# vllm-project/production-stack

Hardware: AMD Instinct MI355X
Metric: output_tokens_per_sec (higher is better)
Workload: dtype bfloat16; 1 GPU; multi-round-qa; model=llama-3-8b, users_per_gpu=320, rounds_per_conversation=10, max_model_len=8192, parallelism=dp1, prefix_caching=True, kv_cache_dtype=auto, quantization=none

## Files before the change

### csrc/bindings.cpp

```cpp
#include <hip/hip_runtime.h>
#include <torch/extension.h>

#include <c10/hip/HIPStream.h>

#include <algorithm>

extern "C" {
int ps_rms_norm(void* out, const void* x, const void* w, float eps, long T,
                int D, hipStream_t stream);
int ps_fused_add_rms_norm(void* x, void* residual, const void* w, float eps,
                          long T, int D, hipStream_t stream);
int ps_rms_norm_fp8(void* out_q, void* out_scale, void* x, void* residual,
                    const void* w, float eps, long T, int D, int fused,
                    hipStream_t stream);
int ps_silu_and_mul_fp8(void* out_q, void* out_scale, const void* x, long T,
                        int D, hipStream_t stream);
void ps_silu_and_mul(void* out, const void* x, long T, int D,
                     hipStream_t stream);
void ps_rope(const void* positions, void* q, void* k, const void* cos_sin,
             long T, int QH, int KH, int HD, int ROT, hipStream_t stream);
void ps_fused_rope_cache(void* qkv, const void* positions, const void* cos_sin,
                         const void* slot_mapping, void* k_cache,
                         void* v_cache, long T, int QH, int KH, int HD,
                         int ROT, long qkv_stride, int BS, int kv_fp8,
                         hipStream_t stream);
int ps_paged_attn_decode(void* out, void* ws_acc, void* ws_ml, const void* q,
                         const void* k_cache, const void* v_cache,
                         const void* block_tables, const void* seq_lens,
                         int num_seqs, int max_blocks, float scale, int KH,
                         int GQ, int head_dim, int block_size, int num_splits,
                         long q_stride, int variant, int kv_fp8, int window,
                         const void* order, hipStream_t stream);
int ps_decode_order(void* order, const void* seq_lens, int S,
                    hipStream_t stream);
int ps_prefill_mfma32_splits(int num_tiles, int KH, int GQ);
int ps_paged_attn_prefill_mfma32(void* out, void* ws_o, void* ws_ml,
                                 long q_tokens, const void* q,
                                 const void* k_cache, const void* v_cache,
                                 const void* block_tables,
                                 const void* tile_info, int num_tiles,
                                 int num_q_heads, int max_blocks,
                                 float scale, int KH, int GQ, int head_dim,
                                 long q_stride, int kv_fp8, int window,
                                 hipStream_t stream);
int ps_paged_attn_prefill_mfma(void* out, const void* q, const void* k_cache,
                               const void* v_cache, const void* block_tables,
                               const void* tile_info, int num_tiles,
                               int num_q_heads, int max_blocks, float scale,
                               int KH, int GQ, int head_dim, long q_stride,
                               int variant, int kv_fp8, int window, hipStream_t stream);
int ps_paged_attn_prefill(void* out, const void* q, const void* k_cache,
                          const void* v_cache, const void* block_tables,
                          const void* token_seq, const void* token_pos,
                          int num_tokens, int num_q_heads, int max_blocks,
                          float scale, int KH, int GQ, int head_dim,
                          int block_size, long q_stride, int window,
                          hipStream_t stream);
void ps_reshape_and_cache(const void* k, const void* v, void* k_cache,
                          void* v_cache, const void* slot_mapping, long T,
                          int KH, int HD, int BS, int kv_fp8,
                          hipStream_t stream);
void ps_greedy_sample(void* out, const void* logits, long R, int V,
                      hipStream_t stream);
void ps_kv_quant(void* out, void* scales, const void* in, long rows, int hd,
                 hipStream_t stream);
void ps_kv_dequant(void* out, const void* in, const void* scales, long rows,
                   int hd, hipStream_t stream);
int ps_skinny_gemm_splits(int M, int N, int K);
int ps_skinny_gemm(void* out_bf16, void* ws, const void* x, const void* w,
                   int M, int N, int K, long x_stride, hipStream_t stream);
int ps_skinny_gemm_fp8_splits(int M, int N, int K);
int ps_skinny_gemm_fp8(void* out_bf16, void* ws, const void* xq,
                       const void* sx, const void* wq, const void* sw, int M,
                       int N, int K, hipStream_t stream);
int ps_quant_fp8_rows(void* out_q, void* out_scale, const void* x, long T,
                      int D, long x_stride, hipStream_t stream);
int ps_gemm8p_splits(int M, int N, int K);
int ps_gemm8p(void* out_bf16, void* ws, const void* x, const void* w, int M,
              int N, int K, long x_stride, hipStream_t stream);
int ps_lora_bgmv(void* out, const void* x, const void* A, const void* B,
                 const void* scale, const void* idx, int T, int IN, int W,
                 int R, long out_stride, long x_stride, int col_off,
                 hipStream_t stream);
int ps_fused_moe_supported(int T, int top_k, int E, int H, int I);
int ps_fused_moe(void* out, void* offsets, void* sorted_pairs, void* act,
                 void* y, const void* x, const void* w_gate_up,
                 const void* w_down, const void* topk_ids, int ids_i64,
                 const void* topk_w, int T, int top_k, int E, int H, int I,
                 hipStream_t stream);
}

at::Tensor cachegen_encode(at::Tensor q);
at::Tensor cachegen_decode(at::Tensor blob, int64_t hd);

namespace {

hipStream_t current_stream() {
  return c10::hip::getCurrentHIPStream().stream();
}

#define CHECK_GPU_BF16(t)                                             \
  TORCH_CHECK((t).is_cuda(), #t " must be on the GPU");               \
  TORCH_CHECK((t).scalar_type() == at::kBFloat16, #t " must be bf16"); \
  TORCH_CHECK((t).is_contiguous(), #t " must be contiguous")

#define CHECK_GPU_DTYPE(t, ty)                                  \
  TORCH_CHECK((t).is_cuda(), #t " must be on the GPU");         \
  TORCH_CHECK((t).scalar_type() == (ty), #t " dtype mismatch"); \
  TORCH_CHECK((t).is_contiguous(), #t " must be contiguous")

void check_fp8_outputs(const at::Tensor& out_q, const at::Tensor& scales,
                       long T, long D) {
  TORCH_CHECK(out_q.is_cuda() && out_q.is_contiguous(),
              "out_q must be GPU-contiguous");
  TORCH_CHECK(out_q.scalar_type() == at::kFloat8_e4m3fn ||
                  out_q.scalar_type() == at::kByte,
              "out_q must be fp8/byte");
  TORCH_CHECK(out_q.dim() == 2 && out_q.size(0) == T && out_q.size(1) == D,
              "out_q must be [", T, ", ", D, "]");
  CHECK_GPU_DTYPE(scales, at::kFloat);
  TORCH_CHECK(scales.numel() == T, "scales must hold one value per row");
}

int rotary_dim(const at::Tensor& cos_sin, int HD) {
  TORCH_CHECK(cos_sin.dim() == 2, "cos_sin must be [max_pos, rot_dim]");
  const long ROT = cos_sin.size(1);
  TORCH_CHECK(ROT >= 0 && ROT % 2 == 0, "rot_dim must be even, got ", ROT);
// ... 101 lines not shown
  const int QH = (int)q.size(1);
  const int HD = (int)q.size(2);
  const int KH = (int)k_cache.size(1);
  const int BS = (int)k_cache.size(2);
  TORCH_CHECK(QH % KH == 0, "GQA group mismatch");
  const int GQ = QH / KH;
  const int max_blocks = (int)block_tables.size(1);
  if (num_splits <= 0) {
    const int target = 2048;
    num_splits = std::min<int64_t>(
        32, std::max<int64_t>(1, target / std::max(1, S * KH)));
  }
  at::Tensor ws_acc, ws_ml;
  void *acc_p = nullptr, *ml_p = nullptr;
  if (num_splits > 1) {
    auto opts = q.options().dtype(at::kFloat);
    ws_acc = at::empty({(long)S * QH * num_splits * HD}, opts);
    ws_ml = at::empty({(long)S * QH * num_splits * 2}, opts);
    acc_p = ws_acc.data_ptr();
    ml_p = ws_ml.data_ptr();
  }
  int rc = ps_paged_attn_decode(
      out.data_ptr(), acc_p, ml_p, q.data_ptr(), k_cache.data_ptr(),
      v_cache.data_ptr(), block_tables.data_ptr(), seq_lens.data_ptr(), S,
      max_blocks, (float)scale, KH, GQ, HD, BS, (int)num_splits,
      q_row_stride(q, HD), (int)variant, kv_fp8, (int)window, order_p,
      current_stream());
  TORCH_CHECK(rc == 0, "unsupported decode config: head_dim=", HD,
              " block_size=", BS, " gqa=", GQ, " variant=", variant);
}

bool decode_order(at::Tensor order, at::Tensor seq_lens) {
  CHECK_GPU_DTYPE(order, at::kInt);
  CHECK_GPU_DTYPE(seq_lens, at::kInt);
  TORCH_CHECK(order.numel() == seq_lens.numel(), "order/seq_lens size");
  return ps_decode_order(order.data_ptr(), seq_lens.data_ptr(),
                         (int)seq_lens.numel(), current_stream()) == 0;
}

void paged_attn_prefill(at::Tensor out, at::Tensor q, at::Tensor k_cache,
                        at::Tensor v_cache, at::Tensor block_tables,
                        at::Tensor token_seq, at::Tensor token_pos,
                        double scale, int64_t window) {
  CHECK_GPU_BF16(out);
  CHECK_GPU_BF16(k_cache);
  CHECK_GPU_BF16(v_cache);
  CHECK_GPU_DTYPE(block_tables, at::kInt);
  CHECK_GPU_DTYPE(token_seq, at::kInt);
  CHECK_GPU_DTYPE(token_pos, at::kInt);
  const int T = (int)q.size(0);
  const int QH = (int)q.size(1);
  const int HD = (int)q.size(2);
  const int KH = (int)k_cache.size(1);
  const int BS = (int)k_cache.size(2);
  TORCH_CHECK(QH % KH == 0, "GQA group mismatch");
  const int GQ = QH / KH;
  const int max_blocks = (int)block_tables.size(1);
  int rc = ps_paged_attn_prefill(
      out.data_ptr(), q.data_ptr(), k_cache.data_ptr(), v_cache.data_ptr(),
      block_tables.data_ptr(), token_seq.data_ptr(), token_pos.data_ptr(), T,
      QH, max_blocks, (float)scale, KH, GQ, HD, BS, q_row_stride(q, HD),
      (int)window, current_stream());
  TORCH_CHECK(rc == 0, "unsupported prefill config: head_dim=", HD,
              " block_size=", BS);
}

void paged_attn_prefill_mfma(at::Tensor out, at::Tensor q,
                             at::Tensor k_cache, at::Tensor v_cache,
                             at::Tensor block_tables, at::Tensor tile_info,
                             double scale, int64_t variant, int64_t window) {
  CHECK_GPU_BF16(out);
  const int kv_fp8 = cache_fp8(k_cache);
  cache_fp8(v_cache);
  CHECK_GPU_DTYPE(block_tables, at::kInt);
  CHECK_GPU_DTYPE(tile_info, at::kInt);
  const int QH = (int)q.size(1);
  const int HD = (int)q.size(2);
  const int KH = (int)k_cache.size(1);
  TORCH_CHECK(QH % KH == 0, "GQA group mismatch");
  TORCH_CHECK(k_cache.size(2) == 16, "mfma prefill needs block_size 16");
  const int GQ = QH / KH;
  const int NT = (int)tile_info.size(0);
  int rc;
  if (variant == 5) {
    const int splits = ps_prefill_mfma32_splits(NT, KH, QH / KH);
    const long T = q.size(0);
    void *ws_o_p = nullptr, *ws_ml_p = nullptr;
    at::Tensor ws_o, ws_ml;
    if (splits > 1) {
      ws_o = at::empty({(long)splits * T * QH * HD},
                       q.options().dtype(at::kFloat));
      ws_ml = at::empty({2L * splits * T * QH},
                        q.options().dtype(at::kFloat));
      ws_o_p = ws_o.data_ptr();
      ws_ml_p = ws_ml.data_ptr();
    }
    rc = ps_paged_attn_prefill_mfma32(
        out.data_ptr(), ws_o_p, ws_ml_p, T, q.data_ptr(),
        k_cache.data_ptr(), v_cache.data_ptr(), block_tables.data_ptr(),
        tile_info.data_ptr(), NT, QH, (int)block_tables.size(1),
        (float)scale, KH, QH / KH, HD, q_row_stride(q, HD), kv_fp8,
        (int)window, current_stream());
  } else {
    rc = ps_paged_attn_prefill_mfma(
        out.data_ptr(), q.data_ptr(), k_cache.data_ptr(),
        v_cache.data_ptr(), block_tables.data_ptr(), tile_info.data_ptr(),
        NT, QH, (int)block_tables.size(1), (float)scale, KH, GQ, HD,
        q_row_stride(q, HD), (int)variant, kv_fp8, (int)window,
        current_stream());
  }
  TORCH_CHECK(rc == 0, "unsupported mfma prefill config: head_dim=", HD);
}

void fused_rope_cache(at::Tensor qkv, at::Tensor positions,
                      at::Tensor cos_sin, at::Tensor slot_mapping,
                      at::Tensor k_cache, at::Tensor v_cache,
                      int64_t q_heads, int64_t head_dim) {
  CHECK_GPU_BF16(qkv);
  CHECK_GPU_DTYPE(positions, at::kInt);
  CHECK_GPU_DTYPE(cos_sin, at::kFloat);
  CHECK_GPU_DTYPE(slot_mapping, at::kLong);
  const int kv_fp8 = cache_fp8(k_cache);
  cache_fp8(v_cache);
  const long T = positions.numel();
  TORCH_CHECK(k_cache.dim() == 4 && v_cache.sizes() == k_cache.sizes() &&
                  v_cache.scalar_type() == k_cache.scalar_type(),
              "k/v cache must both be [NB, KH, BS, HD] of one dtype");
  const int KH = (int)k_cache.size(1);
  const int BS = (int)k_cache.size(2);
  TORCH_CHECK(head_dim > 0 && head_dim % 8 == 0,
              "head_dim must be a positive multiple of 8");
  const int HD = (int)head_dim;
  TORCH_CHECK(k_cache.size(3) == HD, "cache head_dim mismatch");
  const int ROT = rotary_dim(cos_sin, HD);
  TORCH_CHECK(qkv.dim() == 2 && qkv.size(0) == T &&
                  qkv.size(1) == (q_heads + 2 * KH) * HD,
              "qkv must be [T, (q_heads + 2*KH) * head_dim]");
  TORCH_CHECK(slot_mapping.numel() == T, "one slot per token");
  if (T == 0) return;
  ps_fused_rope_cache(qkv.data_ptr(), positions.data_ptr(),
                      cos_sin.data_ptr(), slot_mapping.data_ptr(),
                      k_cache.data_ptr(), v_cache.data_ptr(), T,
                      (int)q_heads, KH, HD, ROT, qkv.stride(0), BS, kv_fp8,
                      current_stream());
}

void reshape_and_cache(at::Tensor k, at::Tensor v, at::Tensor k_cache,
                       at::Tensor v_cache, at::Tensor slot_mapping) {
  CHECK_GPU_BF16(k);
  CHECK_GPU_BF16(v);
  const int kv_fp8 = cache_fp8(k_cache);
  cache_fp8(v_cache);
  CHECK_GPU_DTYPE(slot_mapping, at::kLong);
  const long T = slot_mapping.numel();
  TORCH_CHECK(k_cache.dim() == 4 && v_cache.sizes() == k_cache.sizes() &&
                  v_cache.scalar_type() == k_cache.scalar_type(),
              "k/v cache must both be [NB, KH, BS, HD] of one dtype");
  const int KH = (int)k_cache.size(1);
  const int BS = (int)k_cache.size(2);
  const int HD = (int)k_cache.size(3);
  TORCH_CHECK(HD % 8 == 0, "head_dim must be a multiple of 8");
  TORCH_CHECK(k.numel() == T * KH * HD, "k shape mismatch");
  TORCH_CHECK(v.numel() == T * KH * HD, "v shape mismatch");
  if (T == 0) return;
  ps_reshape_and_cache(k.data_ptr(), v.data_ptr(), k_cache.data_ptr(),
                       v_cache.data_ptr(), slot_mapping.data_ptr(), T, KH, HD,
                       BS, kv_fp8, current_stream());
}

void skinny_gemm(at::Tensor out, at::Tensor x, at::Tensor w) {
  CHECK_GPU_BF16(out);
  TORCH_CHECK(x.is_cuda() && x.scalar_type() == at::kBFloat16,
              "x must be bf16");
  TORCH_CHECK(x.dim() == 2 && x.stride(1) == 1, "x must be 2D row-major");
  CHECK_GPU_BF16(w);
  const int M = (int)x.size(0);
  const int K = (int)x.size(1);
  const int N = (int)w.size(0);
  TORCH_CHECK(w.size(1) == K, "K mismatch");
  const int splits = ps_skinny_gemm_splits(M, N, K);
  TORCH_CHECK(splits > 0, "unsupported skinny gemm shape M=", M, " N=", N,
              " K=", K);
  void* ws_p = nullptr;
  at::Tensor ws;
  if (splits > 1) {
// ... 324 lines not shown
```

### csrc/prefill_mfma.hip

```cpp
#include "ps_common.h"

typedef __attribute__((ext_vector_type(8))) __bf16 ps_mbf16x8;
typedef __attribute__((ext_vector_type(4))) float ps_mf32x4;

PS_DEV ps_mbf16x8 ps_as_mbf16(ps_bf16x8 u) {
  union {
    ps_bf16x8 u16;
    ps_mbf16x8 bf;
  } v;
  v.u16 = u;
  return v.bf;
}

#define PS_CHUNK 64
#define PS_PL_STRIDE 72

template <int HEAD_DIM, int WPS, typename KVT>
__global__ __launch_bounds__(256, WPS) void paged_attn_prefill_mfma_kernel(
    unsigned short* __restrict__ out,
    const unsigned short* __restrict__ q,
    const KVT* __restrict__ k_cache,
    const KVT* __restrict__ v_cache,
    const int* __restrict__ block_tables,
    const int* __restrict__ tile_info,
// ... 175 lines not shown
      for (int r = 0; r < 4; r++) m_new[r] = ps_group_max<16>(m_new[r]);
      constexpr float PS_RESCALE_THR = 11.54f;
      bool grew = false;
#pragma unroll
      for (int r = 0; r < 4; r++)
        grew |= (m_new[r] > m_run[r] + PS_RESCALE_THR) ||
                (m_run[r] == PS_NEG_INF && m_new[r] > PS_NEG_INF);
      if (__any(grew)) {
#pragma unroll
        for (int r = 0; r < 4; r++) {
          const float corr = exp2f(m_run[r] - m_new[r]);
          l_run[r] *= corr;
#pragma unroll
          for (int s = 0; s < 8; s++) o_acc[s][r] *= corr;
          m_run[r] = m_new[r];
        }
      }
      float psum[4] = {0.f, 0.f, 0.f, 0.f};
#pragma unroll
      for (int ct = 0; ct < NCT; ct++) {
#pragma unroll
        for (int r = 0; r < 4; r++) {
          const float p = s_frag[ct][r] > PS_NEG_INF
                              ? exp2f(s_frag[ct][r] - m_run[r])
                              : 0.f;
          s_frag[ct][r] = p;
          psum[r] += p;
        }
      }
#pragma unroll
      for (int r = 0; r < 4; r++) {
        float rs = ps_group_sum<16>(psum[r]);
        l_run[r] += rs;
      }
#pragma unroll
      for (int ct = 0; ct < NCT; ct++)
#pragma unroll
        for (int r = 0; r < 4; r++)
          p_lds[wave][g * 4 + r][ct * 16 + rc] =
              ps_f32_to_bf16(s_frag[ct][r]);
#pragma unroll
      for (int kc = 0; kc < NKC; kc++) {
        ps_mbf16x8 p_frag = ps_as_mbf16(
            *(const ps_bf16x8*)(&p_lds[wave][rc][kc * 32 + g * 8]));
        __builtin_amdgcn_s_setprio(1);
#pragma unroll
        for (int s = 0; s < 8; s++) {
          const int d = s * 16 + rc;
          const int pg2 = (kc * 4 + g) ^ (d & 7);
          ps_mbf16x8 v_frag =
              ps_as_mbf16(*(const ps_bf16x8*)(&v_t[d][pg2 << 3]));
          o_acc[s] = __builtin_amdgcn_mfma_f32_16x16x32_bf16(
              p_frag, v_frag, o_acc[s], 0, 0, 0);
        }
        __builtin_amdgcn_s_setprio(0);
      }
    }
    __syncthreads();
  }

#pragma unroll
  for (int r = 0; r < 4; r++) {
    const int lrow = wave * 16 + g * 4 + r;
    if (lrow >= n_rows) continue;
    const float inv = l_run[r] > 0.f ? 1.f / l_run[r] : 0.f;
    unsigned short* orow = out + ((long)(q_tok0 + lrow) * QH + qh) * D;
#pragma unroll
    for (int s = 0; s < 8; s++)
      orow[s * 16 + rc] = ps_f32_to_bf16(o_acc[s][r] * inv);
  }
}

extern "C" {

int ps_prefill_mfma32_splits(int num_tiles, int KH, int GQ);
int ps_paged_attn_prefill_mfma32(void* out, void* ws_o, void* ws_ml,
                                 long q_tokens, const void* q,
                                 const void* k_cache, const void* v_cache,
                                 const void* block_tables,
                                 const void* tile_info, int num_tiles,
                                 int num_q_heads, int max_blocks,
                                 float scale, int KH, int GQ, int head_dim,
                                 long q_stride, int kv_fp8, int window,
                                 hipStream_t stream);

int ps_paged_attn_prefill_mfma(void* out, const void* q, const void* k_cache,
                               const void* v_cache, const void* block_tables,
                               const void* tile_info, int num_tiles,
                               int num_q_heads, int max_blocks, float scale,
                               int KH, int GQ, int head_dim, long q_stride,
                               int variant, int kv_fp8, int window,
                               hipStream_t stream) {
  if (head_dim != 128) return -1;
  if (variant == 5) {
    return ps_paged_attn_prefill_mfma32(
        out, nullptr, nullptr, 0, q, k_cache, v_cache,
        block_tables, tile_info, num_tiles,
        num_q_heads, max_blocks, scale, KH, GQ, head_dim, q_stride,
        kv_fp8, window, stream);
  }
  const int n_work = num_tiles * num_q_heads;
  dim3 grid(((n_work + 7) / 8) * 8);
#define PS_PREFILL_T(WPS, KVT)                                              \
  paged_attn_prefill_mfma_kernel<128, WPS, KVT><<<grid, 256, 0, stream>>>(  \
      (unsigned short*)out, (const unsigned short*)q,                       \
      (const KVT*)k_cache, (const KVT*)v_cache, (const int*)block_tables,   \
      (const int*)tile_info, max_blocks, scale, KH, GQ, q_stride,           \
      num_q_heads, n_work, window)
  if (kv_fp8) {
    if (variant == 3) PS_PREFILL_T(3, unsigned char);
    else PS_PREFILL_T(4, unsigned char);
  } else {
    if (variant == 3) PS_PREFILL_T(3, unsigned short);
    else PS_PREFILL_T(4, unsigned short);
  }
#undef PS_PREFILL_T
  return 0;
}

}
```

### csrc/prefill_mfma32.hip

```cpp
#include "ps_common.h"

typedef __attribute__((ext_vector_type(8))) __bf16 ps_mbf16x8;
typedef __attribute__((ext_vector_type(16))) float ps_mf32x16;

PS_DEV ps_mbf16x8 ps_as_mbf16_32(ps_bf16x8 u) {
  union {
    ps_bf16x8 u16;
    ps_mbf16x8 bf;
  } v;
  v.u16 = u;
  return v.bf;
}

#define PS_CHUNK32 64
#define PS_TILE32 256

template <int HEAD_DIM, int GQW, typename KVT>
__global__ __launch_bounds__(512, 2) void paged_attn_prefill_mfma32_kernel(
    unsigned short* __restrict__ out,
    float* __restrict__ ws_o,
    float* __restrict__ ws_ml,
    long q_tokens,
    const unsigned short* __restrict__ q,
    const KVT* __restrict__ k_cache,
    const KVT* __restrict__ v_cache,
    const int* __restrict__ block_tables,
    const int* __restrict__ tile_info,
    int max_blocks, float scale, int KH, int GQ, long q_stride,
    int QH, int n_work, int window) {
  const int split = blockIdx.y;
  const int n_splits = gridDim.y;
  using KVTr = ps_kv_traits<KVT>;
  using kvec8 = typename KVTr::vec8;
  using kvec4 = typename KVTr::vec4;
  constexpr int D = HEAD_DIM;
  constexpr int BS = 16;
  constexpr int NKS = D / 16;
  constexpr int ROWH = 8 / GQW;

  const int W = n_work;
  const int cpx = (W + 7) >> 3;
  const int w = (blockIdx.x & 7) * cpx + (blockIdx.x >> 3);
  if (w >= W) return;
  const int n_grp = GQ / GQW;
  const int n_tiles = W / (n_grp * KH);
  const int tile = w % n_tiles;
  const int g_grp = (w / n_tiles) % n_grp;
  const int kvh = w / (n_tiles * n_grp);
  const int seq_row = tile_info[tile * 4 + 0];
  const int q_tok0 = tile_info[tile * 4 + 1];
  const int q_pos0 = tile_info[tile * 4 + 2];
  const int n_rows = tile_info[tile * 4 + 3];

  const int tid = threadIdx.x;
  const int wave = tid >> 6;
  const int lane = tid & 63;
  const int hi = lane >> 5;
  const int rc = lane & 31;
  const int qh = kvh * GQ + g_grp * GQW + (wave / ROWH);
  const int wq0 = (wave % ROWH) * 32;

  const int* bt = block_tables + (long)seq_row * max_blocks;
  const int ctx_limit = q_pos0 + n_rows;
  const int n_pages = (ctx_limit + BS - 1) / BS;
  const int n_chunks = (ctx_limit + PS_CHUNK32 - 1) / PS_CHUNK32;

  __shared__ __align__(16) unsigned short k_lds[PS_CHUNK32][D];
  __shared__ __align__(16) unsigned short v_t[D][PS_CHUNK32];
  __shared__ __align__(16) unsigned short p_lds[8][32][64];

  const int q_row_clamped = min(wq0 + rc, n_rows - 1);
  const unsigned short* qrow =
      q + (long)(q_tok0 + q_row_clamped) * q_stride + (long)qh * D;
  const float qmul = scale * 1.44269504f;
  ps_mbf16x8 q_frag[NKS];
#pragma unroll
  for (int ks = 0; ks < NKS; ks++) {
    ps_bf16x8 qv = *(const ps_bf16x8*)(qrow + ks * 16 + hi * 8);
    ps_bf16x8 qs;
#pragma unroll
    for (int j = 0; j < 8; j++)
      qs[j] = ps_f32_to_bf16(ps_bf16_to_f32(qv[j]) * qmul);
    q_frag[ks] = ps_as_mbf16_32(qs);
  }

  float m_run = PS_NEG_INF, l_run = 0.f;
  ps_mf32x16 o_acc[4];
#pragma unroll
  for (int dt = 0; dt < 4; dt++)
#pragma unroll
    for (int r = 16; r-- > 0;) o_acc[dt][r] = 0.f;

  const int q_pos = q_pos0 + wq0 + rc;
  const int wave_pos_max = q_pos0 + min(wq0 + 31, n_rows - 1);
  const int wave_win_lo =
      window > 0 ? max(0, (q_pos0 + wq0) - window + 1) : 0;

  const int ktok = tid >> 3, kslot = tid & 7;
  const int vtq = tid & 15, vds = tid >> 4;
  auto k_seg_ptr = [&](int chunk) {
    const int tok = chunk * PS_CHUNK32 + ktok;
    const long pg = bt[min(tok / BS, n_pages - 1)];
    return k_cache + ((pg * KH + kvh) * BS + (tok & (BS - 1))) * D +
           kslot * 8;
  };
  auto v_quad_ptr = [&](int chunk) {
    const int tok = chunk * PS_CHUNK32 + vtq * 4;
    const long pg = bt[min(tok / BS, n_pages - 1)];
    return v_cache + ((pg * KH + kvh) * BS + (tok & (BS - 1))) * D + vds * 4;
  };
  kvec8 kstage[2];
  kvec4 vstage[4];
  {
    const KVT* ks = k_seg_ptr(split);
    const KVT* vq = v_quad_ptr(split);
    kstage[0] = *(const kvec8*)ks;
    kstage[1] = *(const kvec8*)(ks + 64);
#pragma unroll
    for (int i = 0; i < 4; i++) vstage[i] = *(const kvec4*)(vq + i * D);
  }

  for (int chunk = split; chunk < n_chunks; chunk += n_splits) {
    const int tok0 = chunk * PS_CHUNK32;
    *(ps_bf16x8*)(&k_lds[ktok][(kslot ^ (ktok & 7)) * 8]) =
        KVTr::to_bf16x8(kstage[0]);
    *(ps_bf16x8*)(&k_lds[ktok][((kslot ^ (ktok & 7)) + 8) * 8]) =
        KVTr::to_bf16x8(kstage[1]);
    {
      const int vo = vtq >> 1;
      const int off = (vtq & 1) * 4;
#pragma unroll
      for (int dd = 0; dd < 4; dd++) {
        const int d = vds * 4 + dd;
        unsigned short r4[4];
#pragma unroll
        for (int i = 0; i < 4; i++) r4[i] = KVTr::to_bf16(vstage[i][dd]);
        *(ps_bf16x4*)(&v_t[d][(vo ^ (d & 7)) * 8 + off]) =
            *(const ps_bf16x4*)r4;
      }
    }
    __syncthreads();
    if (chunk + n_splits < n_chunks) {
      const KVT* ks = k_seg_ptr(chunk + n_splits);
      const KVT* vq = v_quad_ptr(chunk + n_splits);
      kstage[0] = *(const kvec8*)ks;
      kstage[1] = *(const kvec8*)(ks + 64);
#pragma unroll
      for (int i = 0; i < 4; i++) vstage[i] = *(const kvec4*)(vq + i * D);
    }

    const bool wave_active = (wq0 < n_rows) && (tok0 <= wave_pos_max) &&
                             (tok0 + PS_CHUNK32 > wave_win_lo);
    if (wave_active) {
      ps_mf32x16 s_frag[2];
#pragma unroll
      for (int kt = 0; kt < 2; kt++) {
#pragma unroll
        for (int r = 16; r-- > 0;) s_frag[kt][r] = 0.f;
        const int ktok_row = kt * 32 + rc;
        __builtin_amdgcn_s_setprio(1);
#pragma unroll
        for (int ks = 0; ks < NKS; ks++) {
          const int slot = ((ks * 2 + hi) ^ (ktok_row & 7));
          ps_mbf16x8 k_frag = ps_as_mbf16_32(
              *(const ps_bf16x8*)(&k_lds[ktok_row][slot * 8]));
          s_frag[kt] = __builtin_amdgcn_mfma_f32_32x32x16_bf16(
              k_frag, q_frag[ks], s_frag[kt], 0, 0, 0);
        }
        __builtin_amdgcn_s_setprio(0);
      }
      bool full_chunk = (tok0 + PS_CHUNK32 - 1 <= q_pos0 + wq0) &&
                        (wq0 + 31 < n_rows);
      if (window > 0)
        full_chunk = full_chunk && (tok0 >= wave_pos_max - window + 1);
      float m_new = m_run;
      if (full_chunk) {
#pragma unroll
        for (int kt = 0; kt < 2; kt++)
#pragma unroll
          for (int r = 0; r < 16; r++)
            m_new = fmaxf(m_new, s_frag[kt][r]);
      } else {
        const bool row_real = (wq0 + rc) < n_rows;
#pragma unroll
        for (int kt = 0; kt < 2; kt++) {
#pragma unroll
          for (int r = 0; r < 16; r++) {
            const int kv_pos =
                tok0 + kt * 32 + (r & 3) + 8 * (r >> 2) + 4 * hi;
            bool valid = row_real && (kv_pos <= q_pos);
            if (window > 0) valid = valid && (kv_pos > q_pos - window);
            const float sv = valid ? s_frag[kt][r] : PS_NEG_INF;
            s_frag[kt][r] = sv;
            m_new = fmaxf(m_new, sv);
          }
        }
      }
      m_new = fmaxf(m_new, __shfl_xor(m_new, 32));
      constexpr float PS_RESCALE_THR32 = 11.54f;
      const bool grew = (m_new > m_run + PS_RESCALE_THR32) ||
                        (m_run == PS_NEG_INF && m_new > PS_NEG_INF);
      if (__any(grew)) {
        const float corr = exp2f(m_run - m_new);
        l_run *= corr;
        m_run = m_new;
#pragma unroll
        for (int r = 0; r < 16; r++) {
          const int row = (r & 3) + 8 * (r >> 2) + 4 * hi;
          const float c = __shfl(corr, row);
#pragma unroll
          for (int dt = 0; dt < 4; dt++) o_acc[dt][r] *= c;
        }
      }
      float psum = 0.f;
#pragma unroll
      for (int kt = 0; kt < 2; kt++) {
#pragma unroll
        for (int r = 0; r < 16; r++) {
          const float p = s_frag[kt][r] > PS_NEG_INF
                              ? exp2f(s_frag[kt][r] - m_run)
                              : 0.f;
          s_frag[kt][r] = p;
          psum += p;
        }
      }
      l_run += psum + __shfl_xor(psum, 32);
#pragma unroll
      for (int kt = 0; kt < 2; kt++)
#pragma unroll
        for (int qd = 0; qd < 4; qd++) {
          unsigned short p4[4];
#pragma unroll
          for (int j = 0; j < 4; j++)
            p4[j] = ps_f32_to_bf16(s_frag[kt][qd * 4 + j]);
          const int slot = (kt * 4 + qd) ^ (rc & 7);
          *(ps_bf16x4*)(&p_lds[wave][rc][slot * 8 + 4 * hi]) =
              *(const ps_bf16x4*)p4;
        }
#pragma unroll
      for (int kc = 0; kc < 4; kc++) {
        const int pslot = ((kc * 2 + hi) ^ (rc & 7));
        ps_mbf16x8 p_frag = ps_as_mbf16_32(
            *(const ps_bf16x8*)(&p_lds[wave][rc][pslot * 8]));
        __builtin_amdgcn_s_setprio(1);
#pragma unroll
        for (int dt = 0; dt < 4; dt++) {
          const int d = dt * 32 + rc;
          const int vo = (kc * 2 + hi) ^ (d & 7);
          ps_mbf16x8 v_frag =
              ps_as_mbf16_32(*(const ps_bf16x8*)(&v_t[d][vo * 8]));
          o_acc[dt] = __builtin_amdgcn_mfma_f32_32x32x16_bf16(
              p_frag, v_frag, o_acc[dt], 0, 0, 0);
        }
        __builtin_amdgcn_s_setprio(0);
      }
    }
    __syncthreads();
  }

  if (n_splits > 1) {
    if (hi == 0 && wq0 + rc < n_rows) {
      const long t = q_tok0 + wq0 + rc;
      ws_ml[((long)split * q_tokens + t) * QH + qh] = m_run;
      ws_ml[((long)(n_splits + split) * q_tokens + t) * QH + qh] = l_run;
    }
#pragma unroll
    for (int r = 0; r < 16; r++) {
      const int row = (r & 3) + 8 * (r >> 2) + 4 * hi;
      const int lrow = wq0 + row;
      if (lrow >= n_rows) continue;
      float* orow = ws_o +
          (((long)split * q_tokens + q_tok0 + lrow) * QH + qh) * D;
#pragma unroll
      for (int dt = 0; dt < 4; dt++)
        orow[dt * 32 + rc] = o_acc[dt][r];
    }
    return;
  }

  const float inv_own = l_run > 0.f ? 1.f / l_run : 0.f;
#pragma unroll
  for (int r = 0; r < 16; r++) {
    const int row = (r & 3) + 8 * (r >> 2) + 4 * hi;
    const int lrow = wq0 + row;
    const float inv = __shfl(inv_own, row);
    if (lrow >= n_rows) continue;
    unsigned short* orow = out + ((long)(q_tok0 + lrow) * QH + qh) * D;
#pragma unroll
    for (int dt = 0; dt < 4; dt++)
      orow[dt * 32 + rc] = ps_f32_to_bf16(o_acc[dt][r] * inv);
  }
}

__global__ void prefill_split_combine_kernel(
    unsigned short* __restrict__ out,
    const float* __restrict__ ws_o,
    const float* __restrict__ ws_ml,
    long q_tokens, int QH, int n_splits) {
  const long th = blockIdx.x;
  if (th >= q_tokens * QH) return;
  const int d = threadIdx.x;
  float M = PS_NEG_INF;
  for (int s = 0; s < n_splits; s++)
    M = fmaxf(M, ws_ml[(long)s * q_tokens * QH + th]);
  float denom = 0.f, acc = 0.f;
  for (int s = 0; s < n_splits; s++) {
    const float m = ws_ml[(long)s * q_tokens * QH + th];
    const float l = ws_ml[((long)(n_splits + s) * q_tokens) * QH + th];
    const float w = (m > PS_NEG_INF && l > 0.f) ? exp2f(m - M) : 0.f;
    denom += w * l;
    acc += w * ws_o[((long)s * q_tokens * QH + th) * 128 + d];
  }
  out[th * 128 + d] =
      ps_f32_to_bf16(denom > 0.f ? acc / denom : 0.f);
}

extern "C" {

int ps_prefill_mfma32_splits(int num_tiles, int KH, int GQ) {
  int gqw = 1;
  while (gqw < 4 && GQ % (gqw * 2) == 0) gqw *= 2;
  const int n_work = num_tiles * KH * (GQ / gqw);
  if (n_work >= 500) return 1;
  int s = (500 + n_work - 1) / n_work;
  return s > 8 ? 8 : s;
}

int ps_paged_attn_prefill_mfma32(void* out, void* ws_o, void* ws_ml,
                                 long q_tokens, const void* q,
                                 const void* k_cache, const void* v_cache,
                                 const void* block_tables,
                                 const void* tile_info, int num_tiles,
                                 int num_q_heads, int max_blocks,
                                 float scale, int KH, int GQ, int head_dim,
                                 long q_stride, int kv_fp8, int window,
                                 hipStream_t stream) {
  if (head_dim != 128) return -1;
  int gqw = 1;
  while (gqw < 4 && GQ % (gqw * 2) == 0) gqw *= 2;
  const int n_work = num_tiles * KH * (GQ / gqw);
  int splits = ps_prefill_mfma32_splits(num_tiles, KH, GQ);
  if (ws_o == nullptr) splits = 1;
  dim3 grid(((n_work + 7) / 8) * 8, splits);
#define PS_PF32_LAUNCH(GQW, KVT)                                          \
  paged_attn_prefill_mfma32_kernel<128, GQW, KVT>                         \
      <<<grid, 512, 0, stream>>>(                                         \
          (unsigned short*)out, (float*)ws_o, (float*)ws_ml, q_tokens,    \
          (const unsigned short*)q,                                       \
          (const KVT*)k_cache, (const KVT*)v_cache,                       \
          (const int*)block_tables, (const int*)tile_info, max_blocks,    \
          scale, KH, GQ, q_stride, num_q_heads, n_work, window)
  if (kv_fp8) {
    if (gqw == 4) PS_PF32_LAUNCH(4, unsigned char);
    else if (gqw == 2) PS_PF32_LAUNCH(2, unsigned char);
    else PS_PF32_LAUNCH(1, unsigned char);
  } else {
    if (gqw == 4) PS_PF32_LAUNCH(4, unsigned short);
    else if (gqw == 2) PS_PF32_LAUNCH(2, unsigned short);
    else PS_PF32_LAUNCH(1, unsigned short);
  }
#undef PS_PF32_LAUNCH
  if (splits > 1) {
    prefill_split_combine_kernel<<<
        dim3((unsigned)(q_tokens * num_q_heads)), 128, 0, stream>>>(
        (unsigned short*)out, (const float*)ws_o, (const float*)ws_ml,
        q_tokens, num_q_heads, splits);
  }
  return 0;
}

}
```

### production_stack_amd/ops/__init__.py

```python

from __future__ import annotations

import os
from typing import Optional

import torch

from production_stack_amd.ops import reference

try:
    from production_stack_amd import _C
except ImportError:
    _C = None

HAVE_EXT = _C is not None


def _require_ext() -> None:
    if _C is None:
        raise RuntimeError(
            "production_stack_amd._C HIP extension is not built; run "
            "`PYTORCH_ROCM_ARCH=gfx950 python setup.py build_ext --inplace`. "
            "Refusing to fall back to eager PyTorch on GPU."
        )
# ... 79 lines not shown

DECODE_VARIANT = int(os.environ.get("PS_DECODE_VARIANT", "3"))
DECODE_ORDER = os.environ.get("PS_DECODE_ORDER", "1") != "0"


def _check_out(out: torch.Tensor, q: torch.Tensor) -> None:
    if (
        out.shape != q.shape
        or out.dtype != q.dtype
        or out.device != q.device
        or not out.is_contiguous()
    ):
        raise ValueError(
            "out must be contiguous with q's shape, dtype and device"
        )


def paged_attn_decode(
    q: torch.Tensor,
    k_cache: torch.Tensor,
    v_cache: torch.Tensor,
    block_tables: torch.Tensor,
    seq_lens: torch.Tensor,
    scale: float,
    window: int = 0,
    order: Optional[torch.Tensor] = None,
    out: Optional[torch.Tensor] = None,
    variant: Optional[int] = None,
) -> torch.Tensor:
    if out is not None:
        _check_out(out, q)
    if q.is_cuda:
        _require_ext()
        if out is None:
            out = torch.empty(q.shape, dtype=q.dtype, device=q.device)
        _C.paged_attn_decode(
            out, q, k_cache, v_cache, block_tables, seq_lens, scale, 0,
            DECODE_VARIANT if variant is None else variant, window, order
        )
        return out
    res = reference.paged_attn_decode(
        q, k_cache, v_cache, block_tables, seq_lens, scale, window
    )
    if out is None:
        return res
    out.copy_(res)
    return out


def decode_order(seq_lens: torch.Tensor) -> Optional[torch.Tensor]:
    if seq_lens.is_cuda:
        _require_ext()
        order = torch.empty_like(seq_lens)
        if not _C.decode_order(order, seq_lens):
            return None
        return order
    return torch.argsort(-seq_lens, stable=True).int()


def paged_attn_prefill(
    q: torch.Tensor,
    k_cache: torch.Tensor,
    v_cache: torch.Tensor,
    block_tables: torch.Tensor,
    token_seq: torch.Tensor,
    token_pos: torch.Tensor,
    scale: float,
    window: int = 0,
) -> torch.Tensor:
    if q.is_cuda:
        _require_ext()
        out = torch.empty(q.shape, dtype=q.dtype, device=q.device)
        _C.paged_attn_prefill(
            out, q, k_cache, v_cache, block_tables, token_seq, token_pos,
            scale, window
        )
        return out
    return reference.paged_attn_prefill(
        q, k_cache, v_cache, block_tables, token_seq, token_pos, scale,
        window
    )


PREFILL_VARIANT = int(os.environ.get("PS_PREFILL_VARIANT", "5"))


def prefill_tile_rows(num_q_heads: int, num_kv_heads: int) -> int:
    if PREFILL_VARIANT != 5:
        return 64
    gq = max(1, num_q_heads // max(1, num_kv_heads))
    gqw = 1
    while gqw < 4 and gq % (gqw * 2) == 0:
        gqw *= 2
    return 32 * (8 // gqw)


def paged_attn_prefill_mfma(
    q: torch.Tensor,
    k_cache: torch.Tensor,
    v_cache: torch.Tensor,
    block_tables: torch.Tensor,
    tile_info: torch.Tensor,
    scale: float,
    window: int = 0,
    variant: int = None,
    out: Optional[torch.Tensor] = None,
) -> torch.Tensor:
    _require_ext()
    if out is None:
        out = torch.empty(q.shape, dtype=q.dtype, device=q.device)
    else:
        _check_out(out, q)
    v = PREFILL_VARIANT if variant is None else variant
    _C.paged_attn_prefill_mfma(
        out, q, k_cache, v_cache, block_tables, tile_info, scale, v, window
    )
    return out


def greedy_sample(logits: torch.Tensor) -> torch.Tensor:
    if logits.is_cuda:
        _require_ext()
        if logits.dtype != torch.bfloat16:
            return logits.float().argmax(dim=-1)
        out = torch.empty(
            logits.shape[0], dtype=torch.long, device=logits.device
        )
        _C.greedy_sample(out, logits)
        return out
    return reference.greedy_sample(logits)


def kv_quant(x: torch.Tensor) -> tuple:
    if x.is_cuda:
        _require_ext()
        hd = x.shape[-1]
        out = torch.empty(x.shape, dtype=torch.int8, device=x.device)
        scales = torch.empty(
            x.numel() // hd, dtype=torch.float32, device=x.device
        )
        _C.kv_quant(out, scales, x)
        return out, scales
    return reference.kv_quant(x)


def kv_dequant(
    q: torch.Tensor, scales: torch.Tensor, dtype=torch.bfloat16
) -> torch.Tensor:
    if q.is_cuda:
        _require_ext()
        out = torch.empty(q.shape, dtype=dtype, device=q.device)
        _C.kv_dequant(out, q, scales)
        return out
    return reference.kv_dequant(q, scales, dtype)


def skinny_gemm(x: torch.Tensor, w: torch.Tensor) -> torch.Tensor:
    _require_ext()
    out = torch.empty(
        (x.shape[0], w.shape[0]), dtype=torch.bfloat16, device=x.device
    )
    _C.skinny_gemm(out, x, w)
    return out


def cachegen_encode(q: torch.Tensor) -> torch.Tensor:
    if _C is not None and hasattr(_C, "cachegen_encode"):
        return _C.cachegen_encode(q.contiguous().cpu())
    return reference.cachegen_encode(q)


# ... 200 lines not shown
```

Baseline: 5948 tokens/s.

## Add double-buffered prefill attention variant with register-resident P and make it default

Adds variant 6 of the 32x32 MFMA prefill attention kernel. It double-buffers the K/V shared-memory tiles so that one barrier per chunk replaces two, and overlaps staging of the next chunk with compute. It also keeps the softmax probabilities in registers by swapping the MFMA operand order, which removes the P round-trip through LDS and the per-row corr shuffles, and it uses the raw exp2 builtin. The cost is more LDS for the K/V buffers (offset by dropping p_lds), a transposed output layout, and some risk in the edge handling of -inf rows.

```diff
diff --git a/csrc/bindings.cpp b/csrc/bindings.cpp
--- a/csrc/bindings.cpp
+++ b/csrc/bindings.cpp
@@ -42,7 +42,7 @@
                                  int num_q_heads, int max_blocks,
                                  float scale, int KH, int GQ, int head_dim,
                                  long q_stride, int kv_fp8, int window,
-                                 hipStream_t stream);
+                                 int variant, hipStream_t stream);
 int ps_paged_attn_prefill_mfma(void* out, const void* q, const void* k_cache,
                                const void* v_cache, const void* block_tables,
                                const void* tile_info, int num_tiles,
@@ -310,7 +310,7 @@
   const int GQ = QH / KH;
   const int NT = (int)tile_info.size(0);
   int rc;
-  if (variant == 5) {
+  if (variant == 5 || variant == 6) {
     const int splits = ps_prefill_mfma32_splits(NT, KH, QH / KH);
     const long T = q.size(0);
     void *ws_o_p = nullptr, *ws_ml_p = nullptr;
@@ -328,7 +328,7 @@
         k_cache.data_ptr(), v_cache.data_ptr(), block_tables.data_ptr(),
         tile_info.data_ptr(), NT, QH, (int)block_tables.size(1),
         (float)scale, KH, QH / KH, HD, q_row_stride(q, HD), kv_fp8,
-        (int)window, current_stream());
+        (int)window, (int)variant, current_stream());
   } else {
     rc = ps_paged_attn_prefill_mfma(
         out.data_ptr(), q.data_ptr(), k_cache.data_ptr(),
diff --git a/csrc/prefill_mfma.hip b/csrc/prefill_mfma.hip
--- a/csrc/prefill_mfma.hip
+++ b/csrc/prefill_mfma.hip
@@ -281,7 +281,7 @@
                                  int num_q_heads, int max_blocks,
                                  float scale, int KH, int GQ, int head_dim,
                                  long q_stride, int kv_fp8, int window,
-                                 hipStream_t stream);
+                                 int variant, hipStream_t stream);
 
 int ps_paged_attn_prefill_mfma(void* out, const void* q, const void* k_cache,
                                const void* v_cache, const void* block_tables,
@@ -291,12 +291,12 @@
                                int variant, int kv_fp8, int window,
                                hipStream_t stream) {
   if (head_dim != 128) return -1;
-  if (variant == 5) {
+  if (variant == 5 || variant == 6) {
     return ps_paged_attn_prefill_mfma32(
         out, nullptr, nullptr, 0, q, k_cache, v_cache,
         block_tables, tile_info, num_tiles,
         num_q_heads, max_blocks, scale, KH, GQ, head_dim, q_stride,
-        kv_fp8, window, stream);
+        kv_fp8, window, variant, stream);
   }
   const int n_work = num_tiles * num_q_heads;
   dim3 grid(((n_work + 7) / 8) * 8);
diff --git a/csrc/prefill_mfma32.hip b/csrc/prefill_mfma32.hip
--- a/csrc/prefill_mfma32.hip
+++ b/csrc/prefill_mfma32.hip
@@ -15,7 +15,7 @@
 #define PS_CHUNK32 64
 #define PS_TILE32 256
 
-template <int HEAD_DIM, int GQW, typename KVT>
+template <int HEAD_DIM, int GQW, typename KVT, int VAR>
 __global__ __launch_bounds__(512, 2) void paged_attn_prefill_mfma32_kernel(
     unsigned short* __restrict__ out,
     float* __restrict__ ws_o,
@@ -37,6 +37,8 @@
   constexpr int BS = 16;
   constexpr int NKS = D / 16;
   constexpr int ROWH = 8 / GQW;
+  constexpr bool V6 = VAR == 6;
+  constexpr int NBUF = V6 ? 2 : 1;
 
   const int W = n_work;
   const int cpx = (W + 7) >> 3;
@@ -65,9 +67,9 @@
   const int n_pages = (ctx_limit + BS - 1) / BS;
   const int n_chunks = (ctx_limit + PS_CHUNK32 - 1) / PS_CHUNK32;
 
-  __shared__ __align__(16) unsigned short k_lds[PS_CHUNK32][D];
-  __shared__ __align__(16) unsigned short v_t[D][PS_CHUNK32];
-  __shared__ __align__(16) unsigned short p_lds[8][32][64];
+  __shared__ __align__(16) unsigned short k_lds[NBUF][PS_CHUNK32][D];
+  __shared__ __align__(16) unsigned short v_t[NBUF][D][PS_CHUNK32];
+  __shared__ __align__(16) unsigned short p_lds[V6 ? 1 : 8][32][64];
 
   const int q_row_clamped = min(wq0 + rc, n_rows - 1);
   const unsigned short* qrow =
@@ -111,42 +113,52 @@
   };
   kvec8 kstage[2];
   kvec4 vstage[4];
-  {
-    const KVT* ks = k_seg_ptr(split);
-    const KVT* vq = v_quad_ptr(split);
+  auto stage_load = [&](int chunk) {
+    const KVT* ks = k_seg_ptr(chunk);
+    const KVT* vq = v_quad_ptr(chunk);
     kstage[0] = *(const kvec8*)ks;
     kstage[1] = *(const kvec8*)(ks + 64);
 #pragma unroll
     for (int i = 0; i < 4; i++) vstage[i] = *(const kvec4*)(vq + i * D);
-  }
-
+  };
+  auto stage_write = [&](int b) {
+    *(ps_bf16x8*)(&k_lds[b][ktok][(kslot ^ (ktok & 7)) * 8]) =
+        KVTr::to_bf16x8(kstage[0]);
+    *(ps_bf16x8*)(&k_lds[b][ktok][((kslot ^ (ktok & 7)) + 8) * 8]) =
+        KVTr::to_bf16x8(kstage[1]);
+    const int vo = V6 ? (vtq >> 2) * 2 + (vtq & 1) : vtq >> 1;
+    const int off = V6 ? (vtq & 2) * 2 : (vtq & 1) * 4;
+#pragma unroll
+    for (int dd = 0; dd < 4; dd++) {
+      const int d = vds * 4 + dd;
+      unsigned short r4[4];
+#pragma unroll
+      for (int i = 0; i < 4; i++) r4[i] = KVTr::to_bf16(vstage[i][dd]);
+      *(ps_bf16x4*)(&v_t[b][d][(vo ^ (d & 7)) * 8 + off]) =
+          *(const ps_bf16x4*)r4;
+    }
+  };
+  stage_load(split);
+  if constexpr (V6) {
+    stage_write(0);
+    if (split + n_splits < n_chunks) stage_load(split + n_splits);
+  }
+
+  int buf = 0;
   for (int chunk = split; chunk < n_chunks; chunk += n_splits) {
     const int tok0 = chunk * PS_CHUNK32;
-    *(ps_bf16x8*)(&k_lds[ktok][(kslot ^ (ktok & 7)) * 8]) =
-        KVTr::to_bf16x8(kstage[0]);
-    *(ps_bf16x8*)(&k_lds[ktok][((kslot ^ (ktok & 7)) + 8) * 8]) =
-        KVTr::to_bf16x8(kstage[1]);
-    {
-      const int vo = vtq >> 1;
-      const int off = (vtq & 1) * 4;
-#pragma unroll
-      for (int dd = 0; dd < 4; dd++) {
-        const int d = vds * 4 + dd;
-        unsigned short r4[4];
-#pragma unroll
-        for (int i = 0; i < 4; i++) r4[i] = KVTr::to_bf16(vstage[i][dd]);
-        *(ps_bf16x4*)(&v_t[d][(vo ^ (d & 7)) * 8 + off]) =
-            *(const ps_bf16x4*)r4;
-      }
-    }
-    __syncthreads();
-    if (chunk + n_splits < n_chunks) {
-      const KVT* ks = k_seg_ptr(chunk + n_splits);
-      const KVT* vq = v_quad_ptr(chunk + n_splits);
-      kstage[0] = *(const kvec8*)ks;
-      kstage[1] = *(const kvec8*)(ks + 64);
-#pragma unroll
-      for (int i = 0; i < 4; i++) vstage[i] = *(const kvec4*)(vq + i * D);
+    if constexpr (V6) {
+      __syncthreads();
+      if (chunk + n_splits < n_chunks) {
+        stage_write(buf ^ 1);
+        if (chunk + 2 * n_splits < n_chunks)
+          stage_load(chunk + 2 * n_splits);
+      }
+    } else {
+      stage_write(0);
+      __syncthreads();
+      if (chunk + n_splits < n_chunks)
+        stage_load(chunk + n_splits);
     }
 
     const bool wave_active = (wq0 < n_rows) && (tok0 <= wave_pos_max) &&
@@ -163,7 +175,7 @@
         for (int ks = 0; ks < NKS; ks++) {
           const int slot = ((ks * 2 + hi) ^ (ktok_row & 7));
           ps_mbf16x8 k_frag = ps_as_mbf16_32(
-              *(const ps_bf16x8*)(&k_lds[ktok_row][slot * 8]));
+              *(const ps_bf16x8*)(&k_lds[buf][ktok_row][slot * 8]));
           s_frag[kt] = __builtin_amdgcn_mfma_f32_32x32x16_bf16(
               k_frag, q_frag[ks], s_frag[kt], 0, 0, 0);
         }
@@ -204,58 +216,98 @@
         const float corr = exp2f(m_run - m_new);
         l_run *= corr;
         m_run = m_new;
+        if constexpr (V6) {
+#pragma unroll
+          for (int r = 0; r < 16; r++)
+#pragma unroll
+            for (int dt = 0; dt < 4; dt++) o_acc[dt][r] *= corr;
+        } else {
+#pragma unroll
+          for (int r = 0; r < 16; r++) {
+            const int row = (r & 3) + 8 * (r >> 2) + 4 * hi;
+            const float c = __shfl(corr, row);
+#pragma unroll
+            for (int dt = 0; dt < 4; dt++) o_acc[dt][r] *= c;
+          }
+        }
+      }
+      float psum = 0.f;
+      const float m_sub = (V6 && m_run == PS_NEG_INF) ? 0.f : m_run;
+#pragma unroll
+      for (int kt = 0; kt < 2; kt++) {
 #pragma unroll
         for (int r = 0; r < 16; r++) {
-          const int row = (r & 3) + 8 * (r >> 2) + 4 * hi;
-          const float c = __shfl(corr, row);
-#pragma unroll
-          for (int dt = 0; dt < 4; dt++) o_acc[dt][r] *= c;
-        }
-      }
-      float psum = 0.f;
-#pragma unroll
-      for (int kt = 0; kt < 2; kt++) {
-#pragma unroll
-        for (int r = 0; r < 16; r++) {
-          const float p = s_frag[kt][r] > PS_NEG_INF
-                              ? exp2f(s_frag[kt][r] - m_run)
-                              : 0.f;
+          float p;
+          if constexpr (V6)
+            p = __builtin_amdgcn_exp2f(s_frag[kt][r] - m_sub);
+          else
+            p = s_frag[kt][r] > PS_NEG_INF ? exp2f(s_frag[kt][r] - m_run)
+                                           : 0.f;
           s_frag[kt][r] = p;
           psum += p;
         }
       }
       l_run += psum + __shfl_xor(psum, 32);
-#pragma unroll
-      for (int kt = 0; kt < 2; kt++)
-#pragma unroll
-        for (int qd = 0; qd < 4; qd++) {
-          unsigned short p4[4];
-#pragma unroll
-          for (int j = 0; j < 4; j++)
-            p4[j] = ps_f32_to_bf16(s_frag[kt][qd * 4 + j]);
-          const int slot = (kt * 4 + qd) ^ (rc & 7);
-          *(ps_bf16x4*)(&p_lds[wave][rc][slot * 8 + 4 * hi]) =
-              *(const ps_bf16x4*)p4;
-        }
-#pragma unroll
-      for (int kc = 0; kc < 4; kc++) {
-        const int pslot = ((kc * 2 + hi) ^ (rc & 7));
-        ps_mbf16x8 p_frag = ps_as_mbf16_32(
-            *(const ps_bf16x8*)(&p_lds[wave][rc][pslot * 8]));
-        __builtin_amdgcn_s_setprio(1);
-#pragma unroll
-        for (int dt = 0; dt < 4; dt++) {
-          const int d = dt * 32 + rc;
-          const int vo = (kc * 2 + hi) ^ (d & 7);
-          ps_mbf16x8 v_frag =
-              ps_as_mbf16_32(*(const ps_bf16x8*)(&v_t[d][vo * 8]));
-          o_acc[dt] = __builtin_amdgcn_mfma_f32_32x32x16_bf16(
-              p_frag, v_frag, o_acc[dt], 0, 0, 0);
-        }
-        __builtin_amdgcn_s_setprio(0);
-      }
-    }
-    __syncthreads();
+      if constexpr (V6) {
+#pragma unroll
+        for (int g = 0; g < 4; g++) {
+          ps_mbf16x8 p_frag;
+#pragma unroll
+          for (int i = 0; i < 8; i += 2) {
+            const ps_f32x2 p2 = {s_frag[g >> 1][(g & 1) * 8 + i],
+                                 s_frag[g >> 1][(g & 1) * 8 + i + 1]};
+            const ps_rawbf16x2 b2 = __builtin_convertvector(p2, ps_rawbf16x2);
+            p_frag[i] = b2[0];
+            p_frag[i + 1] = b2[1];
+          }
+          __builtin_amdgcn_s_setprio(1);
+#pragma unroll
+          for (int dt = 0; dt < 4; dt++) {
+            const int d = dt * 32 + rc;
+            const int vo = (g * 2 + hi) ^ (d & 7);
+            ps_mbf16x8 v_frag = ps_as_mbf16_32(
+                *(const ps_bf16x8*)(&v_t[buf][d][vo * 8]));
+            o_acc[dt] = __builtin_amdgcn_mfma_f32_32x32x16_bf16(
+                v_frag, p_frag, o_acc[dt], 0, 0, 0);
+          }
+          __builtin_amdgcn_s_setprio(0);
+        }
+      } else {
+#pragma unroll
+        for (int kt = 0; kt < 2; kt++)
+#pragma unroll
+          for (int qd = 0; qd < 4; qd++) {
+            unsigned short p4[4];
+#pragma unroll
+            for (int j = 0; j < 4; j++)
+              p4[j] = ps_f32_to_bf16(s_frag[kt][qd * 4 + j]);
+            const int slot = (kt * 4 + qd) ^ (rc & 7);
+            *(ps_bf16x4*)(&p_lds[wave][rc][slot * 8 + 4 * hi]) =
+                *(const ps_bf16x4*)p4;
+          }
+#pragma unroll
+        for (int kc = 0; kc < 4; kc++) {
+          const int pslot = ((kc * 2 + hi) ^ (rc & 7));
+          ps_mbf16x8 p_frag = ps_as_mbf16_32(
+              *(const ps_bf16x8*)(&p_lds[wave][rc][pslot * 8]));
+          __builtin_amdgcn_s_setprio(1);
+#pragma unroll
+          for (int dt = 0; dt < 4; dt++) {
+            const int d = dt * 32 + rc;
+            const int vo = (kc * 2 + hi) ^ (d & 7);
+            ps_mbf16x8 v_frag =
+                ps_as_mbf16_32(*(const ps_bf16x8*)(&v_t[0][d][vo * 8]));
+            o_acc[dt] = __builtin_amdgcn_mfma_f32_32x32x16_bf16(
+                p_frag, v_frag, o_acc[dt], 0, 0, 0);
+          }
+          __builtin_amdgcn_s_setprio(0);
+        }
+      }
+    }
+    if constexpr (V6)
+      buf ^= 1;
+    else
+      __syncthreads();
   }
 
   if (n_splits > 1) {
@@ -263,6 +315,21 @@
       const long t = q_tok0 + wq0 + rc;
       ws_ml[((long)split * q_tokens + t) * QH + qh] = m_run;
       ws_ml[((long)(n_splits + split) * q_tokens + t) * QH + qh] = l_run;
+    }
+    if constexpr (V6) {
+      if (wq0 + rc < n_rows) {
+        float* orow = ws_o +
+            (((long)split * q_tokens + q_tok0 + wq0 + rc) * QH + qh) * D;
+#pragma unroll
+        for (int dt = 0; dt < 4; dt++)
+#pragma unroll
+          for (int qd = 0; qd < 4; qd++) {
+            const ps_f32x4 o4 = {o_acc[dt][qd * 4], o_acc[dt][qd * 4 + 1],
+                                 o_acc[dt][qd * 4 + 2], o_acc[dt][qd * 4 + 3]};
+            *(ps_f32x4*)(orow + dt * 32 + qd * 8 + hi * 4) = o4;
+          }
+      }
+      return;
     }
 #pragma unroll
     for (int r = 0; r < 16; r++) {
@@ -279,6 +346,23 @@
   }
 
   const float inv_own = l_run > 0.f ? 1.f / l_run : 0.f;
+  if constexpr (V6) {
+    if (wq0 + rc < n_rows) {
+      unsigned short* orow =
+          out + ((long)(q_tok0 + wq0 + rc) * QH + qh) * D;
+#pragma unroll
+      for (int dt = 0; dt < 4; dt++)
+#pragma unroll
+        for (int qd = 0; qd < 4; qd++) {
+          ps_bf16x4 o4;
+#pragma unroll
+          for (int j = 0; j < 4; j++)
+            o4[j] = ps_f32_to_bf16(o_acc[dt][qd * 4 + j] * inv_own);
+          *(ps_bf16x4*)(orow + dt * 32 + qd * 8 + hi * 4) = o4;
+        }
+    }
+    return;
+  }
 #pragma unroll
   for (int r = 0; r < 16; r++) {
     const int row = (r & 3) + 8 * (r >> 2) + 4 * hi;
@@ -334,22 +418,28 @@
                                  int num_q_heads, int max_blocks,
                                  float scale, int KH, int GQ, int head_dim,
                                  long q_stride, int kv_fp8, int window,
-                                 hipStream_t stream) {
+                                 int variant, hipStream_t stream) {
   if (head_dim != 128) return -1;
+  if (variant != 5 && variant != 6) return -1;
   int gqw = 1;
   while (gqw < 4 && GQ % (gqw * 2) == 0) gqw *= 2;
   const int n_work = num_tiles * KH * (GQ / gqw);
   int splits = ps_prefill_mfma32_splits(num_tiles, KH, GQ);
   if (ws_o == nullptr) splits = 1;
   dim3 grid(((n_work + 7) / 8) * 8, splits);
-#define PS_PF32_LAUNCH(GQW, KVT)                                          \
-  paged_attn_prefill_mfma32_kernel<128, GQW, KVT>                         \
+#define PS_PF32_LAUNCH_V(GQW, KVT, VAR)                                   \
+  paged_attn_prefill_mfma32_kernel<128, GQW, KVT, VAR>                    \
       <<<grid, 512, 0, stream>>>(                                         \
           (unsigned short*)out, (float*)ws_o, (float*)ws_ml, q_tokens,    \
           (const unsigned short*)q,                                       \
           (const KVT*)k_cache, (const KVT*)v_cache,                       \
           (const int*)block_tables, (const int*)tile_info, max_blocks,    \
           scale, KH, GQ, q_stride, num_q_heads, n_work, window)
+#define PS_PF32_LAUNCH(GQW, KVT)                                          \
+  do {                                                                    \
+    if (variant == 6) PS_PF32_LAUNCH_V(GQW, KVT, 6);                      \
+    else PS_PF32_LAUNCH_V(GQW, KVT, 5);                                   \
+  } while (0)
   if (kv_fp8) {
     if (gqw == 4) PS_PF32_LAUNCH(4, unsigned char);
     else if (gqw == 2) PS_PF32_LAUNCH(2, unsigned char);
@@ -360,6 +450,7 @@
     else PS_PF32_LAUNCH(1, unsigned short);
   }
 #undef PS_PF32_LAUNCH
+#undef PS_PF32_LAUNCH_V
   if (splits > 1) {
     prefill_split_combine_kernel<<<
         dim3((unsigned)(q_tokens * num_q_heads)), 128, 0, stream>>>(
diff --git a/production_stack_amd/ops/__init__.py b/production_stack_amd/ops/__init__.py
--- a/production_stack_amd/ops/__init__.py
+++ b/production_stack_amd/ops/__init__.py
@@ -185,11 +185,11 @@
     )
 
 
-PREFILL_VARIANT = int(os.environ.get("PS_PREFILL_VARIANT", "5"))
+PREFILL_VARIANT = int(os.environ.get("PS_PREFILL_VARIANT", "6"))
 
 
 def prefill_tile_rows(num_q_heads: int, num_kv_heads: int) -> int:
-    if PREFILL_VARIANT != 5:
+    if PREFILL_VARIANT not in (5, 6):
         return 64
     gq = max(1, num_q_heads // max(1, num_kv_heads))
     gqw = 1
```

Result: faster. 6064 tokens/s (median of 5 runs) (+2.0%).
